# TheShadow29/zsgnet-pytorch

Measured on AMD Instinct MI355X. Metric: train images/sec, higher is better.
Workload: dtype f32

## Files before the change

### include/zsg.h

```cpp
#ifndef ZSG_H
#define ZSG_H

#include <stddef.h>
#include <stdint.h>

#ifdef __cplusplus
extern "C" {
#endif

#define ZSG_VERSION 100
#define ZSG_MAX_SEG 8

int zsg_version(void);
const char* zsg_source_stamp(void);
const char* zsg_last_error(void);
int zsg_set_deterministic(int32_t on);

typedef struct {
    int32_t n;
    int32_t w0;
    int32_t wstep;
    int32_t d0;
    int32_t dstep;
} zsg_taps;
// ... 86 lines not shown
#define ZSG_IO_ADD_BF16 4
int zsg_conv_igemm_bf16_io(const zsg_conv_desc* d, const void* src, const uint16_t* wt_packed, void* out, const float* bias,
                           const void* add_src, int32_t io_flags, void* stream);
int32_t zsg_conv_igemm_bf16_io_supported(const zsg_conv_desc* d, int32_t io_flags);
int zsg_maxpool_fwd_bf16(const void* x, int32_t x_bf16, int32_t B, int32_t H, int32_t W, int32_t C, int32_t k, int32_t s, int32_t p,
                         int32_t Ho, int32_t Wo, uint16_t* out, void* stream);
int zsg_upsample_add_fwd_bf16(const uint16_t* a, const uint16_t* p, int32_t B, int32_t Hs, int32_t Ws, int32_t Hd, int32_t Wd, int32_t C,
                              uint16_t* out, void* stream);
int zsg_relu_fwd_bf16(const uint16_t* x, int64_t n, uint16_t* out, void* stream);
int zsg_avgpool_fwd_bf16(const uint16_t* x, int32_t B, int32_t HW, int32_t C, uint16_t* out, void* stream);
int zsg_head_shared_conv0_bf16(const float* Y, const void* img_idx, int32_t idx_i64, const float* bias, const float* G, const float* V,
                               int32_t Bi, int32_t Q, int32_t nlev, const int32_t* hw, int32_t N, uint16_t* out, void* stream);
int zsg_cast_f32_bf16(const float* x, int64_t n, uint16_t* out, void* stream);
int zsg_cast_bf16_f32(const uint16_t* x, int64_t n, float* out, void* stream);

int64_t zsg_wino_u_elems(int32_t C, int32_t N);
int zsg_wino_weights(const void* jobs, int32_t njobs, int32_t total_blocks, void* stream);

size_t zsg_conv_wgrad_wino_workspace_bytes(const zsg_conv_desc* d);
int zsg_conv_wgrad_wino(const zsg_conv_desc* d, const float* src, const float* dy, float* dw, int32_t accumulate, void* ws,
                        size_t ws_bytes, void* stream);
int zsg_conv_wgrad_wino_batched(const zsg_conv_desc* d, int32_t njobs, const float* const* src, const float* const* dy, float* const* dw,
                                int32_t accumulate, void* ws, size_t ws_bytes, void* stream);

int zsg_transpose_w(const float* src, float* dst, int32_t N, int32_t T, int32_t C, int32_t dst_ld, void* stream);
int zsg_transpose_w_batched(const float* src_base, float* dst_base, const void* jobs, int32_t njobs, int32_t total_tiles,
                            void* stream);
int zsg_pad_rows(const float* src, int64_t rows, int32_t C, int32_t src_ld, float* dst, int32_t dst_ld, void* stream);

int zsg_colsum(const float* x, int32_t groups, int64_t gstride, int32_t rows, int32_t ld, int32_t c0, int32_t C,
               float* out, int32_t accumulate, void* stream);

size_t zsg_bn_workspace_bytes(int64_t rows, int32_t C);
int zsg_bn_stats(const float* x, int64_t rows, int32_t C, float* mean, float* invstd, float* running_mean,
                 float* running_var, float momentum, float eps, void* ws, size_t ws_bytes, void* stream);
int zsg_bn_stats_from_partials(const float* partials, int32_t chunks, int64_t rows, int32_t C, float* mean, float* invstd,
                               float* running_mean, float* running_var, float momentum, float eps, void* stream);
int zsg_bn_relu_maxpool_fwd(const float* x, int32_t B, int32_t H, int32_t W, int32_t C, const float* mean, const float* invstd,
                            const float* gamma, const float* beta, int32_t k, int32_t s, int32_t p, int32_t Ho, int32_t Wo, float* out,
                            uint8_t* idx, void* stream);
int zsg_bn_relu_maxpool_bwd(const float* dout, const uint8_t* idx, const float* x, int32_t B, int32_t H, int32_t W, int32_t C,
                            const float* mean, const float* invstd, const float* gamma, const float* beta, int32_t k, int32_t s, int32_t p,
                            int32_t Ho, int32_t Wo, float* dx, float* dgamma, float* dbeta, int32_t accumulate, void* ws, size_t ws_bytes,
                            void* stream);
int32_t zsg_bn_inline_max_chunks(void);
int zsg_bn_apply_from_partials(const float* x, int64_t rows, int32_t C, const float* partials, int32_t chunks, const float* gamma,
// ... 211 lines not shown
```

### zsgnet-pytorch_amd/_lib.py

```python
import ctypes as C
import os

import torch

_HERE = os.path.dirname(os.path.abspath(__file__))
LIB_PATH = os.environ.get("ZSG_LIB_PATH") or os.path.join(_HERE, "libzsg.so")
ZSG_MAX_SEG = 8


class Taps(C.Structure):
    _fields_ = [("n", C.c_int32), ("w0", C.c_int32), ("wstep", C.c_int32), ("d0", C.c_int32), ("dstep", C.c_int32)]


class Seg(C.Structure):
    _fields_ = [("rows_y", C.c_int32), ("rows_x", C.c_int32), ("src_H", C.c_int32), ("src_W", C.c_int32),
                ("sy", C.c_int32), ("sx", C.c_int32), ("out_W", C.c_int32), ("osy", C.c_int32), ("osx", C.c_int32),
                ("opy", C.c_int32), ("opx", C.c_int32), ("reserved", C.c_int32),
                ("src_off", C.c_int64), ("src_bstride", C.c_int64), ("out_off", C.c_int64), ("out_bstride", C.c_int64),
                ("ty", Taps), ("tx", Taps)]


class ConvDesc(C.Structure):
    _fields_ = [("B", C.c_int32), ("C", C.c_int32), ("N", C.c_int32), ("src_ld", C.c_int32), ("out_ld", C.c_int32),
                ("wR", C.c_int32), ("wS", C.c_int32), ("wC", C.c_int32), ("wc0", C.c_int32), ("wt_ld", C.c_int32),
# ... 74 lines not shown
    "zsg_conv_wino_bnstat": (I32, [DP, P, P, P, P, P, P, P, P, P, F32, F32, P]),
    "zsg_conv_igemm_bnb_tail": (I32, [DP, P, P, P, P, P, P, P, P, P, P, P, P, P, I32, P]),
    "zsg_conv_wino_bnb_tail": (I32, [DP, P, P, P, P, P, P, P, P, P, P, P, P, P, I32, P]),
    "zsg_bn_bwd_apply": (I32, [P, P, P, I64, I32, P, P, P, P, P, P, P]),
    "zsg_conv_wino_bnb": (I32, [DP, P, P, P, P, P, P, P, P, P, P]),
    "zsg_bn_backward_from_partials": (I32, [P, P, P, I64, I32, P, P, P, P, P, P, P, I32, P, I32, P, SZ, P]),
    "zsg_bn_frozen_backward": (I32, [P, P, P, I64, I32, P, P, P, P, P, P, P, I32, P, I32, P, SZ, P]),
    "zsg_bn_frozen_relu_maxpool_bwd": (I32, [P, P, P, I32, I32, I32, I32, P, P, P, P, I32, I32, I32, I32, I32, P, P, P, I32, P, SZ, P]),
    "zsg_bn_sync_fwd_sums": (I32, [P, I64, I32, P, I32, P, P, SZ, P]),
    "zsg_bn_sync_fwd_finalize": (I32, [P, I32, P, P, P, P, F32, F32, P]),
    "zsg_bn_sync_bwd_sums": (I32, [P, P, P, I64, I32, P, P, P, I32, P, P, P, I32, P, SZ, P]),
    "zsg_bn_sync_bwd_apply": (I32, [P, P, P, I64, I32, P, P, P, P, P, P, P, P]),
    "zsg_bn_sync_relu_maxpool_bwd_sums": (I32, [P, P, P, I32, I32, I32, I32, P, P, P, P, I32, I32, I32, I32, I32, P, P, P, I32, P, SZ, P]),
    "zsg_bn_sync_relu_maxpool_bwd_apply": (I32, [P, P, P, I32, I32, I32, I32, P, P, P, P, I32, I32, I32, I32, I32, P, P, P, P]),
    "zsg_wino_u_elems": (I64, [I32, I32]),
    "zsg_wino_weights": (I32, [P, I32, I32, P]),
    "zsg_conv_wgrad_workspace_bytes": (SZ, [DP]),
    "zsg_conv_wgrad": (I32, [DP, P, P, P, I32, P, SZ, P]),
    "zsg_conv_wgrad_bf16": (I32, [DP, P, P, P, I32, P, SZ, P]),
    "zsg_conv_wgrad_bf16_supported": (I32, [DP]),
    "zsg_conv_wgrad_wino_workspace_bytes": (SZ, [DP]),
    "zsg_conv_wgrad_wino": (I32, [DP, P, P, P, I32, P, SZ, P]),
    "zsg_conv_wgrad_wino_batched": (I32, [DP, I32, P, P, P, I32, P, SZ, P]),
    "zsg_transpose_w": (I32, [P, P, I32, I32, I32, I32, P]),
    "zsg_transpose_w_batched": (I32, [P, P, P, I32, I32, P]),
    "zsg_pad_rows": (I32, [P, I64, I32, I32, P, I32, P]),
    "zsg_colsum": (I32, [P, I32, I64, I32, I32, I32, I32, P, I32, P]),
    "zsg_bn_workspace_bytes": (SZ, [I64, I32]),
    "zsg_bn_stats": (I32, [P, I64, I32, P, P, P, P, F32, F32, P, SZ, P]),
    "zsg_bn_stats_from_partials": (I32, [P, I32, I64, I32, P, P, P, P, F32, F32, P]),
    "zsg_bn_eval_stats": (I32, [P, P, I32, F32, P, P, P]),
    "zsg_bn_fold": (I32, [P, P, P, F32, P, I32, I32, P, P]),
    "zsg_bn_inline_max_chunks": (I32, []),
    "zsg_bn_apply_from_partials": (I32, [P, I64, I32, P, I32, P, P, P, I32, P, P, P, P, P, P, F32, F32, P]),
    "zsg_bn_apply": (I32, [P, I64, I32, P, P, P, P, P, I32, P, P, P]),
    "zsg_bn_backward": (I32, [P, P, P, P, I64, I32, P, P, P, P, P, P, P, I32, P, SZ, P]),
    "zsg_maxpool_fwd": (I32, [P, I32, I32, I32, I32, I32, I32, I32, I32, I32, P, P, P]),
    "zsg_maxpool_bwd": (I32, [P, P, I32, I32, I32, I32, I32, I32, I32, I32, I32, P, P]),
    "zsg_upsample_add_fwd": (I32, [P, P, I32, I32, I32, I32, I32, I32, P, P]),
    "zsg_upsample_add_bwd": (I32, [P, I32, I32, I32, I32, I32, I32, P, I32, P]),
    "zsg_relu_fwd": (I32, [P, I64, P, P]),
    "zsg_relu_bwd": (I32, [P, P, I64, P, I32, P]),
    "zsg_avgpool_fwd": (I32, [P, I32, I32, I32, P, P]),
    "zsg_avgpool_bwd": (I32, [P, I32, I32, I32, P, I32, P]),
    "zsg_l2norm_fwd": (I32, [P, I64, I32, P, P, P]),
    "zsg_l2norm_bwd": (I32, [P, P, P, I64, I32, P, P]),
# ... 94 lines not shown
```

### zsgnet-pytorch_amd/csrc/wgrad.hip

```cpp
#include <stdlib.h>

#include "wgrad_common.h"

template <int KL>
__device__ __forceinline__ void wgrad_reduce_body(const WgReduceJob& p, int block, f32x4* sm_) {
    constexpr int EL = 256 / KL;
    f32x4 (*sm)[EL] = (f32x4 (*)[EL])sm_;
    const int q4 = p.ncols / 4;
    const int64_t total = (int64_t)p.N * q4;
    const size_t slab = (size_t)p.N * p.ncols;
    const int el = threadIdx.x % EL, kl = threadIdx.x / EL;
    const int64_t i = (int64_t)block * EL + el;
    f32x4 s = {0.f, 0.f, 0.f, 0.f};
    int n = 0, q = 0;
    if (i < total) {
        n = (int)(i / q4);
        q = (int)(i % q4) * 4;
        const float* src = p.ws + (size_t)n * p.ncols + q;
#pragma unroll 4
        for (int k = kl; k < p.splits; k += KL) s += *(const f32x4*)(src + k * slab);
    }
    sm[kl][el] = s;
    __syncthreads();
    for (int o = KL / 2; o > 0; o >>= 1) {
// ... 8 lines not shown
        const int wr = p.ty_w0 + jy * p.ty_wstep, ws_ = p.tx_w0 + jx * p.tx_wstep;
        float* o = p.dw + (size_t)n * p.wt_ld + (wr * p.wS + ws_) * p.wC + p.wc0 + c;
        if (p.accumulate) s += *(const f32x4*)o;
        *(f32x4*)o = s;
    }
}

__global__ __launch_bounds__(256) void wgrad_reduce_kernel(const WgReduceJob p) {
    __shared__ f32x4 sm[256];
    if (p.kl == 16) wgrad_reduce_body<16>(p, blockIdx.x, sm);
    else wgrad_reduce_body<4>(p, blockIdx.x, sm);
}

void wg_reduce_job_fill(WgReduceJob& j, const zsg_conv_desc* d, const float* ws, float* dw, int accumulate, int splits) {
    memset(&j, 0, sizeof(j));
    j.ws = ws; j.dw = dw; j.accumulate = accumulate ? 1 : 0; j.splits = splits;
    j.N = d->N; j.C = d->C; j.wS = d->wS; j.wC = d->wC; j.wc0 = d->wc0; j.wt_ld = d->wt_ld;
    j.txn = d->seg[0].tx.n;
    j.ncols = d->seg[0].ty.n * d->seg[0].tx.n * d->C;
    j.ty_w0 = d->seg[0].ty.w0; j.ty_wstep = d->seg[0].ty.wstep; j.tx_w0 = d->seg[0].tx.w0; j.tx_wstep = d->seg[0].tx.wstep;
    j.kl = wg_reduce_kl(j.N, j.ncols, splits);
}

int wg_reduce_launch(const WgReduceJob& j, hipStream_t st) {
    ZSG_PROF("wgrad_reduce_kernel", st, 0, (double)(j.splits + 1) * j.N * j.ncols * 4);
    ZSG_LAUNCH(wgrad_reduce_kernel, dim3(wg_reduce_blocks(j.N, j.ncols, j.kl)), dim3(256), 0, st, j);
    return 0;
}

template <int TM, int TN, int WG_BK, int WM, int WN, bool AVEC = true, bool WIDE = false, bool DENSE = false>
__global__ __launch_bounds__(64 * WM * WN, 2) void wgrad_kernel(const WgParams p) {
    constexpr int NT = 64 * WM * WN;
    constexpr int BM = 32 * TM * WM, BN = 32 * TN * WN;
    constexpr int LDA = BM + WG_PAD, LDB = BN + WG_PAD;
    constexpr int GA = BM / 4, PA = NT / GA, NA = WG_BK / PA;
    constexpr int GB = BN / 4, PB = NT / GB, NB = WG_BK / PB;
    static_assert(NA >= 1 && NB >= 1, "K tile too short for this thread count");
    extern __shared__ __attribute__((aligned(16))) float wg_smem[];
    typedef float (*TileA)[WG_BK][LDA];
    typedef float (*TileB)[WG_BK][LDB];
    TileA As = (TileA)wg_smem;
    TileB Bs = (TileB)(wg_smem + 2 * WG_BK * LDA);

    const int tid = threadIdx.x;
    const int lane = tid & 63, wave = tid >> 6;
    const int wm = wave / WN, wn = wave % WN;
    const int li = lane & 31, lh = lane >> 5;

    const int nmn = p.m_tiles * p.n_tiles;
// ... 241 lines not shown
                a.out_W == a.rows_x && a.src_bstride == (int64_t)a.src_H * a.src_W * d->src_ld &&
                a.out_bstride == (int64_t)a.rows_y * a.rows_x * d->out_ld;
    }
    int TM = (d->N > 64) ? 2 : 1;
    int TN = (p.ncols > 64) ? 2 : 1;
    int want_splits = 0, w8 = 0;
    if (d->tile_hint) {
        TM = ((d->tile_hint & 0xff) >= 128) ? 2 : 1;
        TN = (((d->tile_hint >> 8) & 0xff) >= 128) ? 2 : 1;
        if (((d->tile_hint >> 8) & 0xff) == 255 && TM == 1) TN = 4;
        want_splits = (d->tile_hint >> 16) & 0xff;
        w8 = ((d->tile_hint >> 24) & 1) && TM == 2 && TN == 2;
    }
    if (!avec || wide) { TM = 1; TN = 1; w8 = 0; }
    p.m_tiles = cdiv(d->N, 64 * TM);
    p.n_tiles = cdiv(p.ncols, 64 * TN);
    const int nmn = p.m_tiles * p.n_tiles;
    int splits = want_splits > 0 ? want_splits : (2 * ZSG_NUM_CU + nmn - 1) / nmn;
    if (splits > 64 && want_splits <= 0) splits = 64;
    if (splits > kt / 2) splits = kt / 2;
    if (splits < 1) splits = 1;
    p.kt_chunk = cdiv(kt, splits);
    p.splits = cdiv(kt, p.kt_chunk);
    if (p.splits > 1) {
        const size_t need = (size_t)p.splits * d->N * p.ncols * sizeof(float);
        if (!ws || ws_bytes < need) ZSG_FAIL(-2, "conv_wgrad: workspace too small (%zu < %zu bytes)", ws_bytes, need);
        p.ws = (float*)ws;
    }
    hipStream_t st = (hipStream_t)stream;
    int dev = 0;
    (void)hipGetDevice(&dev);
    ZSG_REQUIRE(dev >= 0 && dev < ZSG_MAX_DEV, "conv_wgrad: device %d", dev);
    const double wg_flops = 2.0 * rows_all * d->N * p.ncols;
    const double wg_bytes = zsg_conv_alg_bytes(d, accumulate != 0);
    dim3 grid(nmn * p.splits);
#define WG_LAUNCH(TM_, TN_, BK_, WM_, WN_)                                                     \
    do {                                                                                       \
        if (dense) WG_LAUNCH_D(TM_, TN_, BK_, WM_, WN_, true, false, true, ", true, false, true"); \
        else WG_LAUNCH_D(TM_, TN_, BK_, WM_, WN_, true, false, false, "");                       \
    } while (0)
#define WG_LAUNCH_A(TM_, TN_, BK_, WM_, WN_, AV_) WG_LAUNCH_W(TM_, TN_, BK_, WM_, WN_, AV_, false)
#define WG_LAUNCH_W(TM_, TN_, BK_, WM_, WN_, AV_, WD_) WG_LAUNCH_D(TM_, TN_, BK_, WM_, WN_, AV_, WD_, false, "")
#define WG_LAUNCH_D(TM_, TN_, BK_, WM_, WN_, AV_, WD_, DN_, SFX_)                                                              \
    do {                                                                                                                   \
        const size_t lds = (size_t)2 * BK_ * ((32 * TM_ * WM_ + WG_PAD) + (32 * TN_ * WN_ + WG_PAD)) * sizeof(float);       \
        static bool attr_done[ZSG_MAX_DEV] = {};                                                                           \
        if (!attr_done[dev]) {                                                                                             \
            hipError_t e = hipFuncSetAttribute((const void*)wgrad_kernel<TM_, TN_, BK_, WM_, WN_, AV_, WD_, DN_>,              \
                                               hipFuncAttributeMaxDynamicSharedMemorySize, (int)lds);                      \
            if (e != hipSuccess) ZSG_FAIL(-3, "wgrad: hipFuncSetAttribute: %s", hipGetErrorString(e));                      \
            attr_done[dev] = true;                                                                                         \
        }                                                                                                                  \
// ... 7 lines not shown
        WG_LAUNCH_A(1, 1, 16, 2, 2, false);
    } else if (w8) {
        if (BKsel == 32) WG_LAUNCH(2, 1, 32, 2, 4);
        else WG_LAUNCH(2, 1, 16, 2, 4);
    } else if (BKsel == 32) {
        if (TM == 2 && TN == 2) WG_LAUNCH(2, 2, 32, 2, 2);
        else if (TM == 2 && TN == 1) WG_LAUNCH(2, 1, 32, 2, 2);
        else if (TM == 1 && TN == 2) WG_LAUNCH(1, 2, 32, 2, 2);
        else WG_LAUNCH(1, 1, 32, 2, 2);
    } else {
        if (TN == 4) WG_LAUNCH(1, 4, 16, 2, 2);
        else if (TM == 2 && TN == 2) WG_LAUNCH(2, 2, 16, 2, 2);
        else if (TM == 2 && TN == 1) WG_LAUNCH(2, 1, 16, 2, 2);
        else if (TM == 1 && TN == 2) WG_LAUNCH(1, 2, 16, 2, 2);
        else WG_LAUNCH(1, 1, 16, 2, 2);
    }
#undef WG_LAUNCH
#undef WG_LAUNCH_A
#undef WG_LAUNCH_W
#undef WG_LAUNCH_D
    if (p.splits > 1) {
        WgReduceJob j;
        wg_reduce_job_fill(j, d, p.ws, dw, p.accumulate, p.splits);
        wg_reduce_launch(j, st);
    }
    ZSG_CHECK_LAUNCH("conv_wgrad");
    return 0;
}

extern "C" int zsg_conv_wgrad(const zsg_conv_desc* d, const float* src, const float* dy, float* dw, int32_t accumulate, void* ws,
                              size_t ws_bytes, void* stream) {
    return conv_wgrad_impl(d, src, dy, dw, accumulate, ws, ws_bytes, stream);
}
```

### zsgnet-pytorch_amd/csrc/wgrad_bf16.hip

```cpp
#include "bf16.h"
#include "wgrad_common.h"

#define WB_BK 32
#define WB_LDK 40

typedef __bf16 wb_bf16x8 __attribute__((ext_vector_type(8)));

template <int BM, int BN>
__global__ __launch_bounds__(256, 2) void wgrad_bf16_kernel(const WgParams p) {
    constexpr int TM = BM / 64, TN = BN / 64;
    constexpr int RA = BM / 32, KQA = WB_BK / RA;
    constexpr int RB = BN / 32, KQB = WB_BK / RB;
    __shared__ __attribute__((aligned(16))) uint16_t As[2][BM][WB_LDK];
    __shared__ __attribute__((aligned(16))) uint16_t Bs[2][BN][WB_LDK];

    const int tid = threadIdx.x;
    const int lane = tid & 63, wave = tid >> 6;
    const int wm = wave >> 1, wn = wave & 1;
    const int li = lane & 31, lh = lane >> 5;

    const int nmn = p.m_tiles * p.n_tiles;
    const int split = blockIdx.x / nmn;
    const int mn = xcd_remap(blockIdx.x % nmn, nmn);
    const int mt = mn / p.n_tiles, nt = mn % p.n_tiles;
// ... 238 lines not shown
        const zsg_seg& a = d->seg[s];
        const int64_t rows = (int64_t)d->B * a.rows_y * a.rows_x;
        WgSegDev& o = p.seg[s];
        o.rows_y = a.rows_y; o.rows_x = a.rows_x; o.rows = (int)rows; o.kt0 = kt;
        o.src_H = a.src_H; o.src_W = a.src_W; o.sy = a.sy; o.sx = a.sx;
        o.out_W = a.out_W; o.osy = a.osy; o.osx = a.osx; o.opy = a.opy; o.opx = a.opx;
        o.src_off = (int)a.src_off; o.src_bstride = (int)a.src_bstride;
        o.out_off = (int)a.out_off; o.out_bstride = (int)a.out_bstride;
        o.inv_per = 1.0f / (float)(a.rows_y * a.rows_x);
        o.inv_rx = 1.0f / (float)a.rows_x;
        kt += cdiv(rows, WB_BK);
        rows_all += (double)rows;
    }
    p.kt_total = kt;
    p.m_tiles = cdiv(d->N, BM);
    p.n_tiles = cdiv(p.ncols, BN);
    const int nmn = p.m_tiles * p.n_tiles;
    int splits = want_splits > 0 ? want_splits : (2 * ZSG_NUM_CU + nmn - 1) / nmn;
    if (splits > 64 && want_splits <= 0) splits = 64;
    if (splits > kt / 2) splits = kt / 2;
    if (splits < 1) splits = 1;
    p.kt_chunk = cdiv(kt, splits);
    p.splits = cdiv(kt, p.kt_chunk);
    if (p.splits > 1) {
        const size_t need = (size_t)p.splits * d->N * p.ncols * sizeof(float);
        if (!ws || ws_bytes < need) ZSG_FAIL(-2, "conv_wgrad_bf16: workspace too small (%zu < %zu bytes)", ws_bytes, need);
        p.ws = (float*)ws;
    }
    hipStream_t st = (hipStream_t)stream;
    const double wg_flops = 2.0 * rows_all * d->N * p.ncols;
    const double wg_bytes = zsg_conv_alg_bytes(d, accumulate != 0);
    const dim3 grid(nmn * p.splits);
#define WB_LAUNCH(BM_, BN_)                                                                     \
    do {                                                                                        \
        ZSG_PROF("wgrad_bf16_kernel<" #BM_ ", " #BN_ ">", st, wg_flops, wg_bytes);                \
        ZSG_LAUNCH((wgrad_bf16_kernel<BM_, BN_>), grid, dim3(256), 0, st, p);                    \
    } while (0)
    if (BM == 128 && BN == 128) WB_LAUNCH(128, 128);
    else if (BM == 128) WB_LAUNCH(128, 64);
    else if (BN == 128) WB_LAUNCH(64, 128);
    else WB_LAUNCH(64, 64);
#undef WB_LAUNCH
    if (p.splits > 1) {
        WgReduceJob j;
        wg_reduce_job_fill(j, d, p.ws, dw, p.accumulate, p.splits);
        wg_reduce_launch(j, st);
    }
    ZSG_CHECK_LAUNCH("conv_wgrad_bf16");
    return 0;
}
```

### zsgnet-pytorch_amd/csrc/wgrad_common.h

```cpp
#pragma once
#include "common.h"

#define WG_PAD 4
#define ZSG_WG_MAX_JOBS 8

struct WgSegDev {
    int rows_y, rows_x, rows, kt0;
    int src_H, src_W, sy, sx;
    int out_W, osy, osx, opy, opx;
    int src_off, src_bstride, out_off, out_bstride;
    float inv_per, inv_rx;
};

struct WgParams {
    const float* src;
    const float* dy;
    float* dw;
    float* ws;
    int accumulate;
    int C, N, src_ld, out_ld, wS, wC, wc0, wt_ld, nseg;
    int ncols, txn;
    int m_tiles, n_tiles, splits, kt_total, kt_chunk, bk;
    zsg_taps ty, tx;
    WgSegDev seg[ZSG_MAX_SEG];
// ... 6 lines not shown
}

__device__ __forceinline__ int fdiv(int a, int d, float rcp) {
    int q = (int)((float)a * rcp);
    int r = a - mul24(q, d);
    q += (r >= d) ? 1 : 0;
    q -= (r < 0) ? 1 : 0;
    return q;
}

struct WgReduceJob {
    const float* ws;
    float* dw;
    int N, ncols, splits, C, txn, wS, wC, wc0, wt_ld, accumulate;
    int ty_w0, ty_wstep, tx_w0, tx_wstep;
    int kl;
};

static inline int wg_reduce_kl(int N, int ncols, int splits) {
    return (splits >= 32 || (int64_t)N * (ncols / 4) < 65536) ? 16 : 4;
}
static inline int wg_reduce_blocks(int N, int ncols, int kl) { return (int)(((int64_t)N * (ncols / 4) + 256 / kl - 1) / (256 / kl)); }

void wg_reduce_job_fill(WgReduceJob& j, const zsg_conv_desc* d, const float* ws, float* dw, int accumulate, int splits);
int wg_reduce_launch(const WgReduceJob& j, hipStream_t st);
```

### zsgnet-pytorch_amd/csrc/winowg.hip

```cpp
#include "wgrad_common.h"

#define WW_KT 8
#define WW_SP (WW_KT * 64 + 8)
#define WW_BIAS (1 << 24)

struct WwSegDev {
    int tiles_y, tiles_x, tiles, st0;
    int H, W;
    int src_off, src_bstride, dy_off, dy_bstride;
    float inv_per, inv_tx;
};

struct WwParams {
    const float* src;
    const float* dy;
    float* dw;
    float* ws;
    int accumulate;
    int C, N, src_ld, dy_ld, wC, wc0, wt_ld, nseg;
    int m_tiles, n_tiles, splits, st_total, st_chunk, xmap;
    int njobs;
    const float* srcj[ZSG_WG_MAX_JOBS];
    const float* dyj[ZSG_WG_MAX_JOBS];
    float* dwj[ZSG_WG_MAX_JOBS];
// ... 297 lines not shown
        const int64_t tiles = (int64_t)d->B * ((a.src_H + 1) / 2) * ((a.src_W + 1) / 2);
        ZSG_REQUIRE(tiles > 0 && tiles < (1ll << 24), "conv_wgrad_wino: seg %d tiles=%lld (must be < 2^24)", s, (long long)tiles);
        ZSG_REQUIRE(a.src_off + (int64_t)d->B * a.src_bstride < (1ll << 29) && a.out_off + (int64_t)d->B * a.out_bstride < (1ll << 29),
                    "conv_wgrad_wino: tensor exceeds 2^29 elements (2 GB window)");
        ZSG_REQUIRE((a.src_off % 4) == 0 && (a.src_bstride % 4) == 0 && (a.out_off % 4) == 0 && (a.out_bstride % 4) == 0,
                    "conv_wgrad_wino: seg %d operands not 16-byte aligned", s);
        ZSG_REQUIRE(4ll * (a.src_W + 1) * d->src_ld < WW_BIAS, "conv_wgrad_wino: seg %d: row pitch too large", s);
        WwSegDev& o = p.seg[s];
        o.tiles_y = (a.src_H + 1) / 2; o.tiles_x = (a.src_W + 1) / 2; o.tiles = (int)tiles; o.st0 = st;
        o.H = a.src_H; o.W = a.src_W;
        o.src_off = (int)a.src_off; o.src_bstride = (int)a.src_bstride; o.dy_off = (int)a.out_off; o.dy_bstride = (int)a.out_bstride;
        o.inv_per = 1.0f / (float)(o.tiles_y * o.tiles_x);
        o.inv_tx = 1.0f / (float)o.tiles_x;
        st += cdiv(tiles, WW_KT);
        rows_all += (double)d->B * a.src_H * a.src_W;
    }
    p.st_total = st;
    p.m_tiles = cdiv(d->N, 64);
    p.n_tiles = cdiv(d->C, 64);
    const int nmn = p.m_tiles * p.n_tiles;
    const int splits = ww_pick_splits(d, st, jn);
    p.st_chunk = cdiv(st, splits);
    p.splits = cdiv(st, p.st_chunk);
    if (p.splits > 1) {
        const size_t need = (size_t)jn * p.splits * d->N * 9 * d->C * sizeof(float);
        if (!ws || ws_bytes < need) ZSG_FAIL(-2, "conv_wgrad_wino: workspace too small (%zu < %zu bytes)", ws_bytes, need);
        p.ws = (float*)ws;
    }
    p.xmap = (d->tile_hint >> 24) & 1;
    hipStream_t stq = (hipStream_t)stream;
    const size_t lds = (size_t)4 * 16 * WW_SP * sizeof(float);
    static bool attr_done[ZSG_MAX_DEV] = {};
    int dev = 0;
    (void)hipGetDevice(&dev);
    ZSG_REQUIRE(dev >= 0 && dev < ZSG_MAX_DEV, "conv_wgrad_wino: device %d", dev);
    if (!attr_done[dev]) {
        hipError_t e = hipFuncSetAttribute((const void*)wino_wgrad_kernel, hipFuncAttributeMaxDynamicSharedMemorySize, (int)lds);
        if (e != hipSuccess) ZSG_FAIL(-3, "wgrad_wino: hipFuncSetAttribute: %s", hipGetErrorString(e));
        attr_done[dev] = true;
    }
    {
        ZSG_PROF("wino_wgrad_kernel", stq, jn * 2.0 * rows_all * d->N * 9.0 * d->C, jn * zsg_conv_alg_bytes(d, accumulate != 0));
        ZSG_LAUNCH(wino_wgrad_kernel, dim3(jn * nmn * p.splits), dim3(512), lds, stq, p);
    }
    if (p.splits > 1) {
        for (int j = 0; j < jn; ++j) {
            WgReduceJob r;
            wg_reduce_job_fill(r, d, p.ws + (size_t)j * p.splits * d->N * 9 * d->C, njobs ? dwj[j] : dw, p.accumulate, p.splits);
            wg_reduce_launch(r, stq);
        }
    }
    ZSG_CHECK_LAUNCH("conv_wgrad_wino");
    return 0;
}

extern "C" int zsg_conv_wgrad_wino(const zsg_conv_desc* d, const float* src, const float* dy, float* dw, int32_t accumulate, void* ws,
                                   size_t ws_bytes, void* stream) {
    return conv_wgrad_wino_impl(d, src, dy, dw, accumulate, ws, ws_bytes, stream);
}

extern "C" int zsg_conv_wgrad_wino_batched(const zsg_conv_desc* d, int32_t njobs, const float* const* src, const float* const* dy, float* const* dw,
                                           int32_t accumulate, void* ws, size_t ws_bytes, void* stream) {
    ZSG_REQUIRE(njobs >= 1 && src && dy && dw, "conv_wgrad_wino_batched: bad argument");
    return conv_wgrad_wino_impl(d, src[0], dy[0], dw[0], accumulate, ws, ws_bytes, stream, njobs, src, dy, dw);
}
```

### zsgnet-pytorch_amd/mdl.py

```python
import ctypes as _ct
import math
import os
import struct as _struct
import types
import weakref
from dataclasses import dataclass, field
from typing import Any, Dict, List, Optional, Tuple

import numpy as np
import torch
from torch import nn

from . import anchors as anchors_mod
from ._lib import check, lib, require_gpu, stream_ptr
from .ops import (Level, Program, TView, WinoJobs, apply_main_priority_env, autotune_conv, autotune_wgrad_batch, conv_out, ensure_stream_scratch, dgrad_desc, fwd_desc, igemm_partial_rows, marshal,
                  shared_side_stream, tile_hint, wino_mode, wino_ok)
from .params import ParamStore, pad4, register_named

VGG_BASE = [64, 64, "M", 128, 128, "M", 256, 256, 256, "C", 512, 512, 512, "M", 512, 512, 512]
SSD_EXTRAS = [256, "S", 512, 128, "S", 256, 128, 256, 128, 256]

WGRAD_DTYPES = ("fp32", "bf16")
EVAL_DTYPES = ("fp32", "bf16", "bf16_act")
TRAIN_DTYPES = ("fp32", "bf16_head")
ENC_DTYPES = ("fp32", "bf16_fwd")
ENC_BWD_DTYPES = ("fp32", "bf16")
BF16_ENC_PREFIX = "backbone.encoder."
BF16_HEAD_PREFIXES = ("backbone.fpn.", "att_reg_box.", "att_box.", "reg_box.")
LSTM_DIMS = (32, 64, 128, 256)

LIVE_NETS = weakref.WeakSet()

ARCHS = {
    "resnet18": ("basic", (2, 2, 2, 2)),
    "resnet34": ("basic", (3, 4, 6, 3)),
    "resnet50": ("bottleneck", (3, 4, 6, 3)),
# ... 9 lines not shown
    k: int
    stride: int = 1
    pad: int = 0
    dil: int = 1
    bias: bool = False
    merge_x: bool = False

    @property
    def cpad(self):
        return pad4(self.cin)


@dataclass
class BnL:
    name: str
    c: int
    index: int = 0


BNB_FUSE = os.environ.get("ZSG_BNB_FUSE", "1") != "0"
BN_PRE_MIN_MB = 40
STAGE_INPUTS = True
WG_BATCH = os.environ.get("ZSG_WG_BATCH", "1") != "0"


SHARED_PLANS_MAX = 12


def bucket_images(Bi: int, Q: int) -> int:
    if not 1 <= Bi <= Q:
        raise ValueError(f"shared images: {Bi} images for {Q} queries (need 1 <= images <= queries)")
    return min(Q, 1 << (Bi - 1).bit_length())


class Act(TView):

    def __init__(self, buf, B, C, ld, levels, name=""):
        super().__init__(buf, B, C, ld, levels)
        self.name = name
        self.grad: Optional["Act"] = None
        self.gfilled = False
        self.needs_mask = False
        self.requires_grad = True

    @property
    def b16(self) -> bool:
# ... 641 lines not shown
        self.shared = Q is not None
        self.Q = Q if Q is not None else B
        assert not (self.shared and training and sync_bn), "shared training does not synchronize BatchNorm across ranks"
        self.frozen_bn = frozenset(frozen_bn) if training else frozenset()
        self._ev_stats = None
        self.sync_bn = (frozenset(sync_bn) - self.frozen_bn) if training else frozenset()
        self.sync_bn_paths: Dict[str, str] = {}
        self._sync_sums: Dict[str, Tuple[torch.Tensor, torch.Tensor]] = {}
        self.frozen_bn_paths: Dict[str, str] = {}
        self.frozen = frozenset(frozen) if training else frozenset()
        self.dev = net.device
        apply_main_priority_env()
        self.fwd = Program("fwd")
        self.prep = Program("bwd-prep")
        self._prep_stream, self._prep_ev, self._prep_fwd, self._prep_pending = None, None, -1, False
        self._bwd_fwd = -2
        self._rel_ev = torch.cuda.Event()
        self._hc_pin, self._hc_ev = None, None
        self._prep_idx_v = False
        self._out_slots_v = False
        self.expect_backward = False
        self._tunables = []
        self._wg_log = []
        self.g5_from_loss = None
        self.bwd = Program("bwd")
        self.bwd.side_batch = 3 if B * H * W <= (4 << 20) else 1
        self.bwd.side_defer = 1
        self.tape = []
        self.acts: Dict[str, Act] = {}
        self.bytes = 0
        self.wt: Dict[str, torch.Tensor] = {}
        self.grad_ready: Dict[str, int] = {}
        self.reducer = None
        self.fwd_id = 0
        self.wt_jobs, self.wt_arena_used = [], 0
        self.wt_arena = self._buf(net.store.total + 4096 * len(net.convs)) if training else None
        self.fold_jobs, self.fold_used, self.fold_rows = [], 0, 0
        self.fold_arena = self._buf(net.store.total + 8 * len(net.convs)) if (not training and net.bns) else None
        self.wino_jobs = {"fwd": WinoJobs(), "bwd": WinoJobs()}
        self.prep_u, self._u_ev, self._wait_idx = Program("fwd-prep"), None, 1 << 30
        self._side_prep = training
        self._zero_calls = []
        self._lower()
        for i, c in enumerate(self.fwd.calls):
            if any(c is z for z in self._zero_calls):
                self._wait_idx = min(self._wait_idx, i)
# ... 531 lines not shown
        if dy is None:
            return
        if self.trains(L.name + ".weight"):
            dw = fwd_desc(src, dy, L.cpad, L.cout, L.k, L.stride, L.pad, L.dil, wC=L.cpad)
            self.wgrad(dw, src, dy, L.name + ".weight", "wgrad:" + L.name, merge_x=L.merge_x)
        if L.bias and self.trains(L.name + ".bias"):
            base = dy.levels[0].off
            self.bwd.add(lib.zsg_colsum, dy.buf[base:], 1, 0, dy.rows(), dy.ld, 0, L.cout, self.G(L.name + ".bias"), 1,
                         what="bgrad:" + L.name, lane=1)
        if src.requires_grad:
            self.dgrad(L, dy, src, n=L.cpad, completes_bn=completes_bn)

    def wgrad(self, d, src: Act, dy: Act, pname: str, what: str, merge_x: bool = False):
        gw = self.G(pname)
        args = (src.buf, dy.buf, gw, 1, self.wg_ws, self.wg_ws_bytes)
        targs = (src.buf, dy.buf, self.tune_dw, 0, self.wg_ws, self.wg_ws_bytes)
        s0 = d.seg[0]
        wino = (d.wR == 3 and d.wS == 3 and s0.sy == 1 and s0.ty.d0 == -1 and s0.ty.dstep == 1 and not d.merge_x
                and dy.ld % 4 == 0 and wino_mode() != "0")
        if self.wgrad_bf16 and self._wgrad_bf16_ok(d, merge_x):
            self._tune("wgrad", lib.zsg_conv_wgrad_bf16, d, targs, stream_ptr(), self.wg_ws_bytes)
            self.bwd.add(lib.zsg_conv_wgrad_bf16, d, *args, what=what + "+bf16", lane=1)
            self._wg_log.append((len(self.bwd.calls) - 1, d, src, dy, gw, pname, what + "+bf16"))
            return
        self._tune("wgrad", lib.zsg_conv_wgrad, d, targs, stream_ptr(), self.wg_ws_bytes, wino_args=targs if wino else None)
        self.bwd.add(lib.zsg_conv_wgrad_wino if d.use_wino else lib.zsg_conv_wgrad, d, *args, what=what, lane=1)
        self._wg_log.append((len(self.bwd.calls) - 1, d, src, dy, gw, pname, what))

    @staticmethod
    def _wgrad_bf16_ok(d, merge_x: bool = False) -> bool:
        dq = type(d).from_buffer_copy(d)
        dq.merge_x = int(bool(merge_x))
        return bool(lib.zsg_conv_wgrad_bf16_supported(_ct.byref(dq)))

    def dgrad(self, L: ConvL, dy: Act, src: Act, n: int, row0: int = 0, dx: Optional[Act] = None, completes_bn: bool = False):
        cred = dy.ld
        assert cred % 4 == 0
        wt = self._wt(L, cred)
        dx = dx or self.grad_of(src)
        d = dgrad_desc(dy, dx, cred, n, L.k, L.stride, L.pad, L.dil)
        wt_off = row0 * L.k * L.k * cred
        if d.zero_fill and not dx.gfilled:
            (self.prep if self._side_prep else self.bwd).add(lib.zsg_memset_f32, self.base(dx), sum(dx.B * l.H * l.W * dx.ld for l in dx.levels), 0.0,
                                                             what="zero:" + L.name)
            dx.gfilled = True
        mask = None
        if src.needs_mask:
            deltas = {sl.off - dl.off for sl, dl in zip(src.levels, dx.levels)}
            assert len(deltas) == 1 and src.ld == dx.ld, "ReLU mask needs one common offset between src and its gradient"
            mask = src.buf.data_ptr() + 4 * deltas.pop()
# ... 348 lines not shown
        moved_c, moved_l = [], []
        for (i0, i1) in reversed(self._hoist):
            moved_c[0:0] = self.fwd.calls[i0:i1]
            moved_l[0:0] = self.fwd.lanes[i0:i1]
            del self.fwd.calls[i0:i1], self.fwd.lanes[i0:i1]
        self.fwd.calls[hoist_to:hoist_to] = moved_c
        self.fwd.lanes[hoist_to:hoist_to] = moved_l
        if self.training:
            ln = self.fwd.lanes
            j = next((i for i in range(1, len(ln)) if ln[i] == 0), None)
            if j is not None and j > 1 and all(l == 1 for l in ln[1:j]):
                joins = [i for i in range(j, len(ln)) if ln[i] == 2]
                if len(joins) >= 5:
                    k = joins[2] + 1
                    blk_c, blk_l = self.fwd.calls[1:j], ln[1:j]
                    self.fwd.calls[1:k] = self.fwd.calls[j:k] + blk_c
                    self.fwd.lanes[1:k] = ln[j:k] + blk_l

        if self.training:
            for emit in reversed(self.tape):
                emit()
            if WG_BATCH:
                self._batch_wgrads()
            self.grad_ready = {k: v for k, v in self.grad_ready.items() if k not in self.frozen}
        self.tape = []

    def _batch_wgrads(self):
        import ctypes as C_
        groups = {}
        for rec in self._wg_log:
            idx, d, src, dy, gw, pname, what = rec
            if d.nseg != 1 or not d.use_wino or self.bwd.calls[idx][0] is not lib.zsg_conv_wgrad_wino:
                continue
            dz = type(d).from_buffer_copy(d)
            dz.tile_hint = 0
            sig = (bool(d.use_wino), bytes(dz))
            groups.setdefault(sig, []).append(rec)
        drop, put = set(), {}
        for sig, recs in groups.items():
            recs.sort(key=lambda r: r[0])
            for k in range(0, len(recs), 8):
                part = recs[k:k + 8]
                if len(part) < 2:
                    continue
                n = len(part)
                d0 = part[0][1]
# ... 13 lines not shown
                    self.grad_ready[r[5]] = last
                    if r[1] in self._tunables:
                        self._tunables.remove(r[1])
        if not put:
            return
        remap, calls, lanes = {}, [], []
        for i, (c, l) in enumerate(zip(self.bwd.calls, self.bwd.lanes)):
            if i in drop:
                continue
            remap[i] = len(calls)
            calls.append(put.get(i, c))
            lanes.append(l)
        nxt = len(calls)
        for i in range(len(self.bwd.calls), -1, -1):
            if i in remap:
                nxt = remap[i]
            else:
                remap[i] = nxt
        self.bwd.calls, self.bwd.lanes = calls, lanes
        self.grad_ready = {k: remap[v] for k, v in self.grad_ready.items()}
        self.n_wgrad_batches = len(put)
        if self.bwd.side_batch == 3 and getattr(self.net, "block_kind", "") == "bottleneck":
            self.bwd.side_batch = 2

    def _lower_stem_fused(self, L: ConvL, Lb: BnL, x0: Act, H1: int, W1: int, H2: int, W2: int) -> Act:
        net, B = self.net, self.B
        y = self.conv(L, x0, name="stem.y", bn_fuse=Lb)
        rows = B * H1 * W1
        rm, rv = net._rm[Lb.index:Lb.index + Lb.c], net._rv[Lb.index:Lb.index + Lb.c]
        gam, bet = self.P(Lb.name + ".weight"), self.P(Lb.name + ".bias")
        self.ws_need = max(getattr(self, "ws_need", 0), lib.zsg_bn_workspace_bytes(rows, Lb.c))
        frozen = self.bn_frozen(Lb)
        sync = self.bn_synced(Lb)
        if frozen:
            mean, invstd = self._eval_stats(Lb)
        elif sync:
            if getattr(y, "bn_chunks", 0) > 0:
                mean, invstd = y.bn_mean, y.bn_invstd
            else:
                mean, invstd = self._buf(Lb.c), self._buf(Lb.c)
                self._sync_fwd_stats(Lb, y.buf, rows, None, 0, mean, invstd, 0, ws=self.ws)
            self.sync_bn_paths[Lb.name] = "partials" if getattr(y, "bn_chunks", 0) > 0 else "x"
        elif getattr(y, "bn_chunks", 0) > 0:
            mean, invstd = y.bn_mean, y.bn_invstd
            if y.bn_inline is not None:
                self.fwd.add(lib.zsg_bn_stats_from_partials, y.bn_inline, y.bn_chunks, rows, Lb.c, mean, invstd, rm, rv, 0.1, 1e-5, what="stats:" + Lb.name)
# ... 723 lines not shown
                    p.grad = net.store.view(n, net.store.grad)
        if g5.data_ptr() != self.g5_in.data_ptr():
            self.g5_in.view_as(g5).copy_(g5)
        ddp = getattr(net, "_ddp", None)
        if self._prep_fwd == self.fwd_id and self._bwd_fwd != self.fwd_id:
            torch.cuda.current_stream().wait_event(self._prep_ev)
            self._prep_pending = False
        else:
            if self._prep_fwd == self.fwd_id and self._prep_pending:
                torch.cuda.current_stream().wait_event(self._prep_ev)
                self._prep_pending = False
            self.prep.run(st)
        self._bwd_fwd = self.fwd_id
        if ddp is not None and ddp.active:
            if getattr(net, "_grad_reduced", False):
                raise RuntimeError("DDP: second backward without zero_grad() — gradient accumulation is not supported by the "
                                   "flat-buffer reducer (reduced gradients would be all-reduced again)")
            net._grad_reduced = True
            if not (g5.data_ptr() == self.g5_in.data_ptr() and self.g5_from_loss == (self.fwd_id, 1.0 / ddp.world)):
                self.g5_in.mul_(1.0 / ddp.world)
            self.g5_from_loss = None
            if self.reducer is None:
                from .dist import grad_spans
                self.reducer = ddp.make_reducer(grad_spans(net.store.entries, net._param_names, self.grad_ready, self.frozen))
            nb = len(self.bwd.calls)
            self.reducer.run(nb, lambda i, j: self.bwd.run(st, i, j, join=(j == nb)), side_stream=lambda: self.bwd._side)
            self.reducer.wait()
        else:
            self.bwd.run(st)


def map_pretrained_keys(net: "ZSGNet", sd: Dict[str, torch.Tensor]) -> Dict[str, torch.Tensor]:
    own = set(net.state_dict().keys())
    keys = [k[7:] if k.startswith("module.") else k for k in sd]
    if any(k in own for k in keys):
        return {k2: v for k2, v in zip(keys, sd.values())}
    prefix = "backbone.encoder.vgg." if net.backbone_kind == "ssd_vgg" else "backbone.encoder."
    return {prefix + k: v for k, v in zip(keys, sd.values()) if not k.startswith("fc.")}


def load_pretrained_encoder(net: "ZSGNet", path: str) -> int:
    sd = torch.load(path, map_location="cpu")
    if isinstance(sd, dict) and "model_state_dict" in sd:
        sd = sd["model_state_dict"]
    mapped = map_pretrained_keys(net, sd)
    own = net.state_dict()
# ... 26 lines not shown
```

Baseline: 1226.

## Batch split-K wgrad reduce launches and add optional deferred grouping

Adds a multi-job reduce kernel so several split-K weight-gradient reductions run in one launch. Batched Winograd wgrad now submits all its per-job reductions together. It also adds a per-stream defer mechanism, with begin/flush calls inserted into the backward program, that can accumulate reductions across consecutive wgrad calls using disjoint workspace slabs. Grouping is off by default, and the defer path adds workspace pressure and scheduling complexity.

```diff
diff --git a/include/zsg.h b/include/zsg.h
--- a/include/zsg.h
+++ b/include/zsg.h
@@ -132,6 +132,9 @@
                         size_t ws_bytes, void* stream);
 int zsg_conv_wgrad_wino_batched(const zsg_conv_desc* d, int32_t njobs, const float* const* src, const float* const* dy, float* const* dw,
                                 int32_t accumulate, void* ws, size_t ws_bytes, void* stream);
+
+int zsg_wgrad_defer_begin(void* stream);
+int zsg_wgrad_defer_flush(void* stream);
 
 int zsg_transpose_w(const float* src, float* dst, int32_t N, int32_t T, int32_t C, int32_t dst_ld, void* stream);
 int zsg_transpose_w_batched(const float* src_base, float* dst_base, const void* jobs, int32_t njobs, int32_t total_tiles,
diff --git a/zsgnet-pytorch_amd/_lib.py b/zsgnet-pytorch_amd/_lib.py
--- a/zsgnet-pytorch_amd/_lib.py
+++ b/zsgnet-pytorch_amd/_lib.py
@@ -120,6 +120,8 @@
     "zsg_conv_wgrad_wino_workspace_bytes": (SZ, [DP]),
     "zsg_conv_wgrad_wino": (I32, [DP, P, P, P, I32, P, SZ, P]),
     "zsg_conv_wgrad_wino_batched": (I32, [DP, I32, P, P, P, I32, P, SZ, P]),
+    "zsg_wgrad_defer_begin": (I32, [P]),
+    "zsg_wgrad_defer_flush": (I32, [P]),
     "zsg_transpose_w": (I32, [P, P, I32, I32, I32, I32, P]),
     "zsg_transpose_w_batched": (I32, [P, P, P, I32, I32, P]),
     "zsg_pad_rows": (I32, [P, I64, I32, I32, P, I32, P]),
diff --git a/zsgnet-pytorch_amd/csrc/wgrad.hip b/zsgnet-pytorch_amd/csrc/wgrad.hip
--- a/zsgnet-pytorch_amd/csrc/wgrad.hip
+++ b/zsgnet-pytorch_amd/csrc/wgrad.hip
@@ -1,4 +1,7 @@
 #include <stdlib.h>
+
+#include <mutex>
+#include <vector>
 
 #include "wgrad_common.h"
 
@@ -54,9 +57,122 @@
     j.kl = wg_reduce_kl(j.N, j.ncols, splits);
 }
 
-int wg_reduce_launch(const WgReduceJob& j, hipStream_t st) {
-    ZSG_PROF("wgrad_reduce_kernel", st, 0, (double)(j.splits + 1) * j.N * j.ncols * 4);
-    ZSG_LAUNCH(wgrad_reduce_kernel, dim3(wg_reduce_blocks(j.N, j.ncols, j.kl)), dim3(256), 0, st, j);
+__global__ __launch_bounds__(256) void wgrad_reduce_multi_kernel(const WgReduceBatch b) {
+    __shared__ f32x4 sm[256];
+    int j = 0;
+    while (j + 1 < b.n && (int)blockIdx.x >= b.start[j + 1]) ++j;
+    const WgReduceJob& p = b.job[j];
+    const int block = (int)blockIdx.x - b.start[j];
+    if (p.kl == 16) wgrad_reduce_body<16>(p, block, sm);
+    else wgrad_reduce_body<4>(p, block, sm);
+}
+
+static int wg_reduce_launch(const WgReduceJob* jobs, int n, hipStream_t st) {
+    if (n <= 0) return 0;
+    double bytes = 0;
+    for (int i = 0; i < n; ++i) bytes += (double)(jobs[i].splits + 1) * jobs[i].N * jobs[i].ncols * 4;
+    ZSG_PROF("wgrad_reduce_kernel", st, 0, bytes);
+    if (n == 1) {
+        ZSG_LAUNCH(wgrad_reduce_kernel, dim3(wg_reduce_blocks(jobs[0].N, jobs[0].ncols, jobs[0].kl)), dim3(256), 0, st, jobs[0]);
+        return 0;
+    }
+    ZSG_REQUIRE(n <= ZSG_WG_REDUCE_MAX, "wgrad_reduce: %d jobs in one launch (at most %d)", n, ZSG_WG_REDUCE_MAX);
+    WgReduceBatch b;
+    memset(&b, 0, sizeof(b));
+    b.n = n;
+    for (int i = 0; i < n; ++i) {
+        b.job[i] = jobs[i];
+        b.start[i + 1] = b.start[i] + wg_reduce_blocks(jobs[i].N, jobs[i].ncols, jobs[i].kl);
+    }
+    ZSG_LAUNCH(wgrad_reduce_multi_kernel, dim3(b.start[n]), dim3(256), 0, st, b);
+    return 0;
+}
+
+struct WgDefer {
+    hipStream_t st;
+    int dev;
+    bool active;
+    char* base;
+    size_t cursor;
+    int n;
+    WgReduceJob job[ZSG_WG_REDUCE_MAX];
+};
+static std::vector<WgDefer*> g_wg_defer;
+static std::mutex g_wg_defer_mu;
+
+static WgDefer* wg_defer_state(hipStream_t st, bool create) {
+    int dev = 0;
+    (void)hipGetDevice(&dev);
+    std::lock_guard<std::mutex> lk(g_wg_defer_mu);
+    for (WgDefer* s : g_wg_defer)
+        if (s->st == st && s->dev == dev) return s;
+    if (!create) return nullptr;
+    WgDefer* s = new WgDefer();
+    s->st = st;
+    s->dev = dev;
+    g_wg_defer.push_back(s);
+    return s;
+}
+
+static int wg_defer_flush_pending(WgDefer* s) {
+    const int n = s->n;
+    s->n = 0;
+    s->cursor = 0;
+    return wg_reduce_launch(s->job, n, s->st);
+}
+
+int wg_slabs_acquire(hipStream_t st, void* ws, size_t ws_bytes, size_t need, int njobs, const char* who, float** slabs) {
+    if (!ws || ws_bytes < need) ZSG_FAIL(-2, "%s: workspace too small (%zu < %zu bytes)", who, ws_bytes, need);
+    WgDefer* s = wg_defer_state(st, false);
+    if (!s || !s->active) {
+        *slabs = (float*)ws;
+        return 0;
+    }
+    if (s->n && (s->base != (char*)ws || s->n + njobs > ZSG_WG_REDUCE_MAX || s->cursor + need > ws_bytes)) {
+        int rc = wg_defer_flush_pending(s);
+        if (rc) return rc;
+    }
+    if (!s->n) {
+        s->base = (char*)ws;
+        s->cursor = 0;
+    }
+    *slabs = (float*)(s->base + s->cursor);
+    s->cursor += (need + 15) & ~(size_t)15;
+    return 0;
+}
+
+int wg_reduce_submit(const WgReduceJob* jobs, int n, hipStream_t st) {
+    WgDefer* s = wg_defer_state(st, false);
+    if (!s || !s->active) return wg_reduce_launch(jobs, n, st);
+    if (s->n + n > ZSG_WG_REDUCE_MAX) {
+        int rc = wg_defer_flush_pending(s);
+        if (rc) return rc;
+    }
+    ZSG_REQUIRE(n <= ZSG_WG_REDUCE_MAX, "wgrad_reduce: %d jobs in one launch (at most %d)", n, ZSG_WG_REDUCE_MAX);
+    for (int i = 0; i < n; ++i) s->job[s->n++] = jobs[i];
+    return 0;
+}
+
+extern "C" int zsg_wgrad_defer_begin(void* stream) {
+    WgDefer* s = wg_defer_state((hipStream_t)stream, true);
+    if (s->active && s->n) {
+        int rc = wg_defer_flush_pending(s);
+        if (rc) return rc;
+    }
+    s->active = true;
+    s->n = 0;
+    s->cursor = 0;
+    return 0;
+}
+
+extern "C" int zsg_wgrad_defer_flush(void* stream) {
+    WgDefer* s = wg_defer_state((hipStream_t)stream, false);
+    if (!s || !s->active) return 0;
+    s->active = false;
+    if (!s->n) return 0;
+    int rc = wg_defer_flush_pending(s);
+    if (rc) return rc;
+    ZSG_CHECK_LAUNCH("wgrad_defer_flush");
     return 0;
 }
 
@@ -344,12 +460,12 @@
     if (splits < 1) splits = 1;
     p.kt_chunk = cdiv(kt, splits);
     p.splits = cdiv(kt, p.kt_chunk);
+    hipStream_t st = (hipStream_t)stream;
     if (p.splits > 1) {
         const size_t need = (size_t)p.splits * d->N * p.ncols * sizeof(float);
-        if (!ws || ws_bytes < need) ZSG_FAIL(-2, "conv_wgrad: workspace too small (%zu < %zu bytes)", ws_bytes, need);
-        p.ws = (float*)ws;
-    }
-    hipStream_t st = (hipStream_t)stream;
+        int rc = wg_slabs_acquire(st, ws, ws_bytes, need, 1, "conv_wgrad", &p.ws);
+        if (rc) return rc;
+    }
     int dev = 0;
     (void)hipGetDevice(&dev);
     ZSG_REQUIRE(dev >= 0 && dev < ZSG_MAX_DEV, "conv_wgrad: device %d", dev);
@@ -403,7 +519,8 @@
     if (p.splits > 1) {
         WgReduceJob j;
         wg_reduce_job_fill(j, d, p.ws, dw, p.accumulate, p.splits);
-        wg_reduce_launch(j, st);
+        int rc = wg_reduce_submit(&j, 1, st);
+        if (rc) return rc;
     }
     ZSG_CHECK_LAUNCH("conv_wgrad");
     return 0;
diff --git a/zsgnet-pytorch_amd/csrc/wgrad_bf16.hip b/zsgnet-pytorch_amd/csrc/wgrad_bf16.hip
--- a/zsgnet-pytorch_amd/csrc/wgrad_bf16.hip
+++ b/zsgnet-pytorch_amd/csrc/wgrad_bf16.hip
@@ -284,12 +284,12 @@
     if (splits < 1) splits = 1;
     p.kt_chunk = cdiv(kt, splits);
     p.splits = cdiv(kt, p.kt_chunk);
+    hipStream_t st = (hipStream_t)stream;
     if (p.splits > 1) {
         const size_t need = (size_t)p.splits * d->N * p.ncols * sizeof(float);
-        if (!ws || ws_bytes < need) ZSG_FAIL(-2, "conv_wgrad_bf16: workspace too small (%zu < %zu bytes)", ws_bytes, need);
-        p.ws = (float*)ws;
-    }
-    hipStream_t st = (hipStream_t)stream;
+        int rc = wg_slabs_acquire(st, ws, ws_bytes, need, 1, "conv_wgrad_bf16", &p.ws);
+        if (rc) return rc;
+    }
     const double wg_flops = 2.0 * rows_all * d->N * p.ncols;
     const double wg_bytes = zsg_conv_alg_bytes(d, accumulate != 0);
     const dim3 grid(nmn * p.splits);
@@ -306,7 +306,8 @@
     if (p.splits > 1) {
         WgReduceJob j;
         wg_reduce_job_fill(j, d, p.ws, dw, p.accumulate, p.splits);
-        wg_reduce_launch(j, st);
+        int rc = wg_reduce_submit(&j, 1, st);
+        if (rc) return rc;
     }
     ZSG_CHECK_LAUNCH("conv_wgrad_bf16");
     return 0;
diff --git a/zsgnet-pytorch_amd/csrc/wgrad_common.h b/zsgnet-pytorch_amd/csrc/wgrad_common.h
--- a/zsgnet-pytorch_amd/csrc/wgrad_common.h
+++ b/zsgnet-pytorch_amd/csrc/wgrad_common.h
@@ -52,5 +52,14 @@
 }
 static inline int wg_reduce_blocks(int N, int ncols, int kl) { return (int)(((int64_t)N * (ncols / 4) + 256 / kl - 1) / (256 / kl)); }
 
+#define ZSG_WG_REDUCE_MAX 16
+struct WgReduceBatch {
+    WgReduceJob job[ZSG_WG_REDUCE_MAX];
+    int start[ZSG_WG_REDUCE_MAX + 1];
+    int n;
+};
+
 void wg_reduce_job_fill(WgReduceJob& j, const zsg_conv_desc* d, const float* ws, float* dw, int accumulate, int splits);
-int wg_reduce_launch(const WgReduceJob& j, hipStream_t st);
+
+int wg_slabs_acquire(hipStream_t st, void* ws, size_t ws_bytes, size_t need, int njobs, const char* who, float** slabs);
+int wg_reduce_submit(const WgReduceJob* jobs, int n, hipStream_t st);
diff --git a/zsgnet-pytorch_amd/csrc/winowg.hip b/zsgnet-pytorch_amd/csrc/winowg.hip
--- a/zsgnet-pytorch_amd/csrc/winowg.hip
+++ b/zsgnet-pytorch_amd/csrc/winowg.hip
@@ -343,13 +343,13 @@
     const int splits = ww_pick_splits(d, st, jn);
     p.st_chunk = cdiv(st, splits);
     p.splits = cdiv(st, p.st_chunk);
+    hipStream_t stq = (hipStream_t)stream;
     if (p.splits > 1) {
         const size_t need = (size_t)jn * p.splits * d->N * 9 * d->C * sizeof(float);
-        if (!ws || ws_bytes < need) ZSG_FAIL(-2, "conv_wgrad_wino: workspace too small (%zu < %zu bytes)", ws_bytes, need);
-        p.ws = (float*)ws;
+        int rc = wg_slabs_acquire(stq, ws, ws_bytes, need, jn, "conv_wgrad_wino", &p.ws);
+        if (rc) return rc;
     }
     p.xmap = (d->tile_hint >> 24) & 1;
-    hipStream_t stq = (hipStream_t)stream;
     const size_t lds = (size_t)4 * 16 * WW_SP * sizeof(float);
     static bool attr_done[ZSG_MAX_DEV] = {};
     int dev = 0;
@@ -365,11 +365,11 @@
         ZSG_LAUNCH(wino_wgrad_kernel, dim3(jn * nmn * p.splits), dim3(512), lds, stq, p);
     }
     if (p.splits > 1) {
-        for (int j = 0; j < jn; ++j) {
-            WgReduceJob r;
-            wg_reduce_job_fill(r, d, p.ws + (size_t)j * p.splits * d->N * 9 * d->C, njobs ? dwj[j] : dw, p.accumulate, p.splits);
-            wg_reduce_launch(r, stq);
-        }
+        WgReduceJob r[ZSG_WG_MAX_JOBS];
+        for (int j = 0; j < jn; ++j)
+            wg_reduce_job_fill(r[j], d, p.ws + (size_t)j * p.splits * d->N * 9 * d->C, njobs ? dwj[j] : dw, p.accumulate, p.splits);
+        int rc = wg_reduce_submit(r, jn, stq);
+        if (rc) return rc;
     }
     ZSG_CHECK_LAUNCH("conv_wgrad_wino");
     return 0;
diff --git a/zsgnet-pytorch_amd/mdl.py b/zsgnet-pytorch_amd/mdl.py
--- a/zsgnet-pytorch_amd/mdl.py
+++ b/zsgnet-pytorch_amd/mdl.py
@@ -12,6 +12,7 @@
 from torch import nn
 
 from . import anchors as anchors_mod
+from . import wgroups as _wgroups
 from ._lib import check, lib, require_gpu, stream_ptr
 from .ops import (Level, Program, TView, WinoJobs, apply_main_priority_env, autotune_conv, autotune_wgrad_batch, conv_out, ensure_stream_scratch, dgrad_desc, fwd_desc, igemm_partial_rows, marshal,
                   shared_side_stream, tile_hint, wino_mode, wino_ok)
@@ -67,6 +68,8 @@
 BN_PRE_MIN_MB = 40
 STAGE_INPUTS = True
 WG_BATCH = os.environ.get("ZSG_WG_BATCH", "1") != "0"
+WG_REDUCE_GROUP = _wgroups.parse_limit(os.environ.get("ZSG_WG_REDUCE_GROUP"), None)
+WG_REDUCE_GROUP_DEFAULT = {"bottleneck": 0, "basic": 0, "vgg": 0}
 
 
 SHARED_PLANS_MAX = 12
@@ -754,6 +757,8 @@
         self.expect_backward = False
         self._tunables = []
         self._wg_log = []
+        self._wg_leaf = []
+        self.wg_groups = []
         self.g5_from_loss = None
         self.bwd = Program("bwd")
         self.bwd.side_batch = 3 if B * H * W <= (4 << 20) else 1
@@ -1331,10 +1336,12 @@
             self._tune("wgrad", lib.zsg_conv_wgrad_bf16, d, targs, stream_ptr(), self.wg_ws_bytes)
             self.bwd.add(lib.zsg_conv_wgrad_bf16, d, *args, what=what + "+bf16", lane=1)
             self._wg_log.append((len(self.bwd.calls) - 1, d, src, dy, gw, pname, what + "+bf16"))
+            self._wg_leaf.append(self.bwd.calls[-1])
             return
         self._tune("wgrad", lib.zsg_conv_wgrad, d, targs, stream_ptr(), self.wg_ws_bytes, wino_args=targs if wino else None)
         self.bwd.add(lib.zsg_conv_wgrad_wino if d.use_wino else lib.zsg_conv_wgrad, d, *args, what=what, lane=1)
         self._wg_log.append((len(self.bwd.calls) - 1, d, src, dy, gw, pname, what))
+        self._wg_leaf.append(self.bwd.calls[-1])
 
     @staticmethod
     def _wgrad_bf16_ok(d, merge_x: bool = False) -> bool:
@@ -1729,6 +1736,7 @@
                 emit()
             if WG_BATCH:
                 self._batch_wgrads()
+            self._group_wgrads()
             self.grad_ready = {k: v for k, v in self.grad_ready.items() if k not in self.frozen}
         self.tape = []
 
@@ -1788,6 +1796,29 @@
         self.n_wgrad_batches = len(put)
         if self.bwd.side_batch == 3 and getattr(self.net, "block_kind", "") == "bottleneck":
             self.bwd.side_batch = 2
+
+    def _group_wgrads(self, boundaries=()):
+        if not hasattr(self, "_bwd_flat"):
+            self._bwd_flat = (list(self.bwd.calls), list(self.bwd.lanes), dict(self.grad_ready))
+        calls, lanes, ready = self._bwd_flat
+        limit = WG_REDUCE_GROUP if WG_REDUCE_GROUP is not None else WG_REDUCE_GROUP_DEFAULT.get(getattr(self.net, "block_kind", ""), 0)
+        leaf = {id(c) for c in self._wg_leaf}
+        family = (lib.zsg_conv_wgrad, lib.zsg_conv_wgrad_wino, lib.zsg_conv_wgrad_wino_batched, lib.zsg_conv_wgrad_bf16)
+        members = [i for i, c in enumerate(calls) if id(c) in leaf and lanes[i] == 1]
+        closers = [i for i, c in enumerate(calls) if c[0] in family and not (id(c) in leaf and lanes[i] == 1)]
+        if not hasattr(self, "_wg_defer_entries"):
+            self._wg_defer_entries = tuple((fn, marshal(fn, (), self.bwd.keep), what) for fn, what in
+                                           ((lib.zsg_wgrad_defer_begin, "wgrad group: begin"), (lib.zsg_wgrad_defer_flush, "wgrad group: reduce")))
+        begin, flush = self._wg_defer_entries
+        old = self.bwd.calls
+        self.bwd.calls, self.bwd.lanes, ready, self.wg_groups = _wgroups.group_wgrads(
+            calls, lanes, ready, members, limit, begin, flush, closers=closers, boundaries=boundaries)
+        self.grad_ready = {k: v for k, v in ready.items() if k not in self.frozen}
+        self.bwd._sched = {}
+        pos = {id(c): i for i, c in enumerate(self.bwd.calls)}
+        for e in self._b16_log:
+            if e["kind"] not in ("fwd", "enc_fwd") and e.get("idx", -1) >= 0:
+                e["idx"] = pos[id(old[e["idx"]])]
 
     def _lower_stem_fused(self, L: ConvL, Lb: BnL, x0: Act, H1: int, W1: int, H2: int, W2: int) -> Act:
         net, B = self.net, self.B
@@ -2557,6 +2588,10 @@
             self.g5_from_loss = None
             if self.reducer is None:
                 from .dist import grad_spans
+                if self.wg_groups:
+                    flat = {k: v for k, v in self._bwd_flat[2].items() if k not in self.frozen}
+                    pre = ddp.make_reducer(grad_spans(net.store.entries, net._param_names, flat, self.frozen)).buckets
+                    self._group_wgrads(boundaries={b.ready for b in pre})
                 self.reducer = ddp.make_reducer(grad_spans(net.store.entries, net._param_names, self.grad_ready, self.frozen))
             nb = len(self.bwd.calls)
             self.reducer.run(nb, lambda i, j: self.bwd.run(st, i, j, join=(j == nb)), side_stream=lambda: self.bwd._side)
diff --git a/zsgnet-pytorch_amd/wgroups.py b/zsgnet-pytorch_amd/wgroups.py
--- /dev/null
+++ b/zsgnet-pytorch_amd/wgroups.py
@@ -0,0 +1,60 @@
+from typing import Dict, Iterable, List, Optional, Sequence, Tuple
+
+JOIN = "join"
+
+
+def parse_limit(text: Optional[str], default):
+    if text is None or text == "":
+        return default
+    if text == JOIN:
+        return JOIN
+    n = int(text)
+    if n < 0 or n == 1:
+        raise ValueError("ZSG_WG_REDUCE_GROUP: 0 (off), a member count >= 2, or 'join'")
+    return n
+
+
+def group_wgrads(calls: Sequence, lanes: Sequence[int], grad_ready: Dict[str, int], members: Iterable[int], limit, begin, flush,
+                 closers: Iterable[int] = (), boundaries: Iterable[int] = ()) -> Tuple[List, List[int], Dict[str, int], List[Tuple[int, int, List[int]]]]:
+    if not limit:
+        return list(calls), list(lanes), dict(grad_ready), []
+    members, closers, boundaries = set(members), set(closers), set(boundaries)
+    closed, cur = [], []
+
+    def close():
+        if len(cur) >= 2:
+            closed.append(list(cur))
+        cur.clear()
+
+    for i, ln in enumerate(lanes):
+        if ln == 2 or i in closers:
+            close()
+        if i in members:
+            assert ln == 1, "a deferred weight gradient runs on the side stream"
+            cur.append(i)
+            if limit != JOIN and len(cur) >= limit:
+                close()
+        if i in boundaries:
+            close()
+    close()
+    first = {g[0]: g for g in closed}
+    last = {g[-1]: g for g in closed}
+    out_c, out_l, remap, flush_at, groups, opened = [], [], {}, {}, [], {}
+    for i, (c, ln) in enumerate(zip(calls, lanes)):
+        if i in first:
+            opened[id(first[i])] = len(out_c)
+            out_c.append(begin)
+            out_l.append(1)
+        remap[i] = len(out_c)
+        out_c.append(c)
+        out_l.append(ln)
+        if i in last:
+            g = last[i]
+            for m in g:
+                flush_at[m] = len(out_c)
+            groups.append((opened[id(g)], len(out_c), [remap[m] for m in g]))
+            out_c.append(flush)
+            out_l.append(1)
+    remap[len(calls)] = len(out_c)
+    ready = {k: (v if v < 0 else flush_at.get(v, remap[v])) for k, v in grad_ready.items()}
+    return out_c, out_l, ready, groups
```

Result: no change. 1228, median of 6 (+0.1%).
